# feinanshan/TDNet

Measured on AMD Instinct MI355X. Metric: frames/sec (td4-psp18, 1024x2048, full-resolution logits), higher is better.
Workload: dtype f32; 1 GPU; td4-psp18, 1024x2048 Cityscapes-shaped synthetic stream, 3-frame feature cache, 1 clip per GPU; parallelism=clip-parallel x1, RCCL weight broadcast only, target_fps_per_gpu=30

## Files before the change

include/tdnet.h:

```cpp
#ifndef TDNET_H
#define TDNET_H

#include <stddef.h>
#include <stdint.h>

#ifdef __cplusplus
extern "C" {
#endif

typedef struct tdnet tdnet_t;

typedef struct tdnet_cfg {
    int32_t model;
    int32_t backbone;
    int32_t nclass;
    int32_t height;
    int32_t width;
    int32_t device;
} tdnet_cfg;

#define TDNET_WINOGRAD_DEFAULT 3
#define TDNET_ATTENTION_DEFAULT 2
#define TDNET_FUSION_LN_STATS 2
#define TDNET_FUSION_LN_IN_HEAD 4
#define TDNET_FUSION_A_DIRECT 32
#define TDNET_FUSION_DMA_LOADERS 8192
#define TDNET_FUSION_DMA_NARROW 32768
#define TDNET_FUSION_STEM_ROWS 65536
#define TDNET_FUSION_CONV_GROUPS 131072
#define TDNET_FUSION_CLS_IN_HEAD 262144
#define TDNET_FUSION_SPLIT_NARROW 524288
#define TDNET_FUSION_LATE_CHAIN 1048576
#define TDNET_FUSION_PPM_FOLD 2097152
#define TDNET_OVERLAP_CHAINS 1
#define TDNET_OVERLAP_LOWREG_TRANSFORMS 2
#define TDNET_OVERLAP_CHAINS_ANY_SIZE 4
#define TDNET_OVERLAP_GEMM_DMA 8
#define TDNET_OVERLAP_VW_SHIFT 4
#define TDNET_OVERLAP_VW_MASK 0x30
#define TDNET_FUSION_DEFAULT (TDNET_FUSION_LN_STATS | TDNET_FUSION_LN_IN_HEAD | TDNET_FUSION_A_DIRECT | TDNET_FUSION_DMA_LOADERS | TDNET_FUSION_DMA_NARROW | \
                              TDNET_FUSION_STEM_ROWS | TDNET_FUSION_CONV_GROUPS | TDNET_FUSION_CLS_IN_HEAD | TDNET_FUSION_SPLIT_NARROW | TDNET_FUSION_LATE_CHAIN | TDNET_FUSION_PPM_FOLD)
#define TDNET_FUSION_MASK TDNET_FUSION_DEFAULT
#define TDNET_OVERLAP_DEFAULT (TDNET_OVERLAP_CHAINS | TDNET_OVERLAP_GEMM_DMA | (2 << TDNET_OVERLAP_VW_SHIFT))
#define TDNET_OVERLAP_MASK (TDNET_OVERLAP_CHAINS | TDNET_OVERLAP_LOWREG_TRANSFORMS | TDNET_OVERLAP_CHAINS_ANY_SIZE | TDNET_OVERLAP_GEMM_DMA | TDNET_OVERLAP_VW_MASK)
typedef struct tdnet_opts {
    int32_t winograd;
    int32_t precision;
    int32_t pipeline;
    int32_t gemm_persistent;
    int32_t reserved0;
    int32_t attention;
    int32_t fusion;
    int32_t overlap;
    int32_t reserved[8];
} tdnet_opts;
void tdnet_opts_default(tdnet_opts* o);

typedef struct tdnet_arch {
    int32_t dilated;
    int32_t multi_grid;
    int32_t reserved[6];
} tdnet_arch;
void tdnet_arch_default(tdnet_arch* a);

int  tdnet_create(const tdnet_cfg* cfg, tdnet_t** out);
int  tdnet_create_opts(const tdnet_cfg* cfg, const tdnet_opts* opts , tdnet_t** out);
int  tdnet_create_arch(const tdnet_cfg* cfg, const tdnet_arch* arch , const tdnet_opts* opts ,
                       tdnet_t** out);
int  tdnet_get_opts(const tdnet_t* h, tdnet_opts* out);
int  tdnet_get_arch(const tdnet_t* h, tdnet_arch* out);
int  tdnet_feature_dims(const tdnet_t* h, int* height, int* width);
void tdnet_destroy(tdnet_t* h);

int  tdnet_set_weight(tdnet_t* h, const char* name, const float* host, size_t count);
int  tdnet_finalize_weights(tdnet_t* h);
int  tdnet_create_shared(const tdnet_t* weights_of, const tdnet_opts* opts , tdnet_t** out);
int  tdnet_warmup(tdnet_t* h, void* stream);
int  tdnet_memory_bytes(const tdnet_t* h, size_t* weights_bytes, size_t* handle_bytes);

int  tdnet_forward(tdnet_t* h, const float* img_nchw_dev, int pos_id, float* logits_nchw_dev, void* stream);
int  tdnet_argmax(tdnet_t* h, const float* logits_nchw_dev, int32_t* labels_dev, void* stream);
int  tdnet_forward_labels(tdnet_t* h, const float* img_nchw_dev, int pos_id, int32_t* labels_dev, void* stream);
int  tdnet_set_input_u8(tdnet_t* h, int src_height, int src_width, const double* mean , const double* std );
int  tdnet_forward_u8(tdnet_t* h, const uint8_t* img_hwc_dev, int pos_id, float* logits_nchw_dev, void* stream);
int  tdnet_forward_u8_labels(tdnet_t* h, const uint8_t* img_hwc_dev, int pos_id, uint8_t* labels_dev , void* stream);
int  tdnet_argmax_u8(tdnet_t* h, const float* logits_nchw_dev, uint8_t* labels_dev, void* stream);
#define TDNET_YUV_BT601_LIMITED 0
#define TDNET_YUV_BT709_LIMITED 1
#define TDNET_YUV_BT601_FULL 2
#define TDNET_YUV_BT709_FULL 3
int  tdnet_set_input_nv12(tdnet_t* h, int src_height, int src_width, int pitch, size_t uv_offset, int standard,
                          const double* mean , const double* std );
#define TDNET_PIX_RGB24  0
#define TDNET_PIX_BGR24  1
// ... 65 lines not shown
```

tdnet_amd/_capi.py:

```python
import ctypes
import os

_HERE = os.path.dirname(os.path.abspath(__file__))
DEFAULT_LIB = os.path.join(_HERE, "lib", "libtdnet_hip.so")
TEST_LIB = os.path.join(_HERE, "lib", "libtdnet_hip_test.so")

c_float_p = ctypes.POINTER(ctypes.c_float)
c_void_p = ctypes.c_void_p


class TdnetCfg(ctypes.Structure):
    _fields_ = [("model", ctypes.c_int32), ("backbone", ctypes.c_int32), ("nclass", ctypes.c_int32),
                ("height", ctypes.c_int32), ("width", ctypes.c_int32), ("device", ctypes.c_int32)]


class TdnetOpts(ctypes.Structure):
    _fields_ = [("winograd", ctypes.c_int32), ("precision", ctypes.c_int32), ("pipeline", ctypes.c_int32),
                ("gemm_persistent", ctypes.c_int32), ("reserved0", ctypes.c_int32), ("attention", ctypes.c_int32),
                ("fusion", ctypes.c_int32), ("overlap", ctypes.c_int32), ("reserved", ctypes.c_int32 * 8)]

    def as_dict(self):
        return {k: getattr(self, k) for k, _ in self._fields_ if not k.startswith("reserved")}


# ... 46 lines not shown
    "tdnet_forward_u8": (ctypes.c_int, [c_void_p, c_void_p, ctypes.c_int, c_void_p, c_void_p]),
    "tdnet_forward_u8_labels": (ctypes.c_int, [c_void_p, c_void_p, ctypes.c_int, c_void_p, c_void_p]),
    "tdnet_argmax_u8": (ctypes.c_int, [c_void_p, c_void_p, c_void_p, c_void_p]),
    "tdnet_encode_u8": (ctypes.c_int, [c_void_p, c_void_p, ctypes.c_int, c_void_p]),
    "tdnet_propagate_labels_u8": (ctypes.c_int, [c_void_p, c_void_p, c_void_p]),
    "tdnet_set_output_rgb": (ctypes.c_int, [c_void_p, ctypes.c_int, ctypes.c_int, c_void_p, ctypes.c_int]),
    "tdnet_forward_rgb": (ctypes.c_int, [c_void_p, c_void_p, ctypes.c_int, c_void_p, c_void_p]),
    "tdnet_forward_u8_rgb": (ctypes.c_int, [c_void_p, c_void_p, ctypes.c_int, c_void_p, c_void_p]),
    "tdnet_labels_rgb": (ctypes.c_int, [c_void_p, c_void_p, c_void_p, c_void_p]),
    "tdnet_propagate_rgb": (ctypes.c_int, [c_void_p, c_void_p, c_void_p]),
    "tdnet_set_output_overlay": (ctypes.c_int, [c_void_p, c_void_p, ctypes.c_int]),
    "tdnet_forward_u8_overlay": (ctypes.c_int, [c_void_p, c_void_p, ctypes.c_int, c_void_p, c_void_p]),
    "tdnet_labels_overlay": (ctypes.c_int, [c_void_p, c_void_p, c_void_p, c_void_p, c_void_p]),
    "tdnet_propagate_overlay": (ctypes.c_int, [c_void_p, c_void_p, c_void_p, c_void_p]),
    "tdnet_set_output_view": (ctypes.c_int, [c_void_p, c_view_p]),
    "tdnet_set_score": (ctypes.c_int, [c_void_p, c_void_p]),
    "tdnet_forward_score": (ctypes.c_int, [c_void_p, c_void_p, ctypes.c_int, c_void_p, c_void_p, c_void_p]),
    "tdnet_forward_u8_score": (ctypes.c_int, [c_void_p, c_void_p, ctypes.c_int, c_void_p, c_void_p, c_void_p]),
    "tdnet_propagate_score": (ctypes.c_int, [c_void_p, c_void_p, c_void_p, c_void_p]),
    "tdnet_labels_score": (ctypes.c_int, [c_void_p, c_void_p, c_void_p, c_void_p]),
    "tdnet_score_reset": (ctypes.c_int, [c_void_p, c_void_p]),
    "tdnet_score_export": (ctypes.c_int, [c_void_p, c_void_p, c_void_p]),
    "tdnet_score_read": (ctypes.c_long, [c_void_p, c_void_p, ctypes.c_size_t, c_void_p]),
    "tdnet_set_confidence": (ctypes.c_int, [c_void_p, ctypes.c_int, ctypes.c_int]),
    "tdnet_forward_labels_conf": (ctypes.c_int, [c_void_p, c_void_p, ctypes.c_int, c_void_p, c_void_p, c_void_p]),
    "tdnet_forward_u8_labels_conf": (ctypes.c_int, [c_void_p, c_void_p, ctypes.c_int, c_void_p, c_void_p, c_void_p]),
    "tdnet_propagate_labels_conf": (ctypes.c_int, [c_void_p, c_void_p, c_void_p, c_void_p]),
    "tdnet_logits_conf": (ctypes.c_int, [c_void_p, c_void_p, c_void_p, c_void_p, c_void_p]),
    "tdnet_reset": (ctypes.c_int, [c_void_p]),
    "tdnet_fifo_len": (ctypes.c_int, [c_void_p]),
    "tdnet_encode": (ctypes.c_int, [c_void_p, c_void_p, ctypes.c_int, c_void_p]),
    "tdnet_propagate": (ctypes.c_int, [c_void_p, c_void_p, c_void_p]),
    "tdnet_propagate_labels": (ctypes.c_int, [c_void_p, c_void_p, c_void_p]),
    "tdnet_cache_dims": (ctypes.c_int, [c_void_p, ctypes.POINTER(ctypes.c_int), ctypes.POINTER(ctypes.c_int), ctypes.POINTER(ctypes.c_int)]),
    "tdnet_cache_export": (ctypes.c_int, [c_void_p, c_void_p, c_void_p, c_void_p, c_void_p]),
    "tdnet_cache_push": (ctypes.c_int, [c_void_p, c_void_p, c_void_p, c_void_p, c_void_p]),
    "tdnet_get_stage": (ctypes.c_long, [c_void_p, ctypes.c_char_p, c_void_p, ctypes.c_size_t]),
    "tdnet_flops_per_frame": (ctypes.c_double, [c_void_p]),
    "tdnet_set_profiling": (ctypes.c_int, [c_void_p, ctypes.c_int]),
    "tdnet_last_ms": (ctypes.c_double, [c_void_p, ctypes.c_int]),
    "tdnet_last_flops": (ctypes.c_double, [c_void_p, ctypes.c_int]),
    "tdnet_last_launches": (ctypes.c_double, [c_void_p, ctypes.c_int]),
    "tdnet_last_error": (ctypes.c_char_p, []),
    "tdnet_version": (ctypes.c_char_p, []),
}


TEST_SYMBOLS = {
    "tdnet_bench_mfma_peak": (ctypes.c_double, [ctypes.c_int, ctypes.c_int, c_void_p]),
    "tdnet_bench_conv": (ctypes.c_double, [ctypes.c_int] * 9 + [c_opts_p, c_void_p]),
    "tdnet_op_conv2d": (ctypes.c_int, [c_void_p, ctypes.c_int, ctypes.c_int, ctypes.c_int, c_void_p, c_void_p, ctypes.c_int,
                                       ctypes.c_int, ctypes.c_int, ctypes.c_int, c_void_p, ctypes.c_int, c_opts_p, ctypes.c_int,
                                       c_void_p, c_void_p]),
    "tdnet_op_conv2d_f16io": (ctypes.c_int, [c_void_p, ctypes.c_int, ctypes.c_int, ctypes.c_int, c_void_p, c_void_p, ctypes.c_int,
                                             ctypes.c_int, ctypes.c_int, ctypes.c_int, c_void_p, ctypes.c_int, ctypes.c_int,
                                             c_void_p, c_void_p]),
    "tdnet_op_conv2d_f16mix": (ctypes.c_int, [c_void_p, ctypes.c_int, ctypes.c_int, ctypes.c_int, c_void_p, c_void_p, ctypes.c_int,
                                              ctypes.c_int, ctypes.c_int, ctypes.c_int, c_void_p, ctypes.c_int, ctypes.c_int, ctypes.c_int,
                                              ctypes.c_int, c_void_p, c_void_p]),
    "tdnet_op_conv_group_f16": (ctypes.c_int, [ctypes.c_int] + [c_void_p] * 12 + [ctypes.c_int] * 4 + [ctypes.POINTER(ctypes.c_int), c_void_p]),
    "tdnet_op_cache_subsample": (ctypes.c_int, [c_void_p, c_void_p] + [ctypes.c_int] * 4 + [c_void_p, c_void_p, c_void_p]),
    "tdnet_op_conv1x1_rows": (ctypes.c_int, [c_void_p, ctypes.c_int, ctypes.c_int, ctypes.c_int, c_void_p, c_void_p, ctypes.c_int, ctypes.c_int,
                                             c_opts_p, ctypes.c_int, ctypes.c_int, c_void_p, c_void_p]),
    "tdnet_op_maxpool": (ctypes.c_int, [c_void_p, ctypes.c_int, ctypes.c_int, ctypes.c_int, ctypes.c_int, c_void_p, c_void_p]),
    "tdnet_op_stem_f16": (ctypes.c_int, [c_void_p, ctypes.c_int, ctypes.c_int, c_void_p, c_void_p, ctypes.c_int, c_void_p, c_void_p]),
    "tdnet_op_stem": (ctypes.c_int, [c_void_p, ctypes.c_int, ctypes.c_int, c_void_p, c_void_p, c_opts_p, c_void_p, c_void_p]),
    "tdnet_op_attention": (ctypes.c_int, [c_void_p, c_void_p, c_void_p, c_void_p, c_void_p, ctypes.c_int, ctypes.c_int,
                                          ctypes.c_int, ctypes.c_int, c_void_p, c_void_p, c_void_p, c_void_p, c_void_p]),
    "tdnet_op_layernorm_hw": (ctypes.c_int, [c_void_p, ctypes.c_int, ctypes.c_int, c_void_p, c_void_p, c_void_p, c_void_p]),
    "tdnet_op_layernorm_hw_f16": (ctypes.c_int, [c_void_p, ctypes.c_int, ctypes.c_int, c_void_p, c_void_p, c_void_p, c_void_p]),
    "tdnet_op_ppm": (ctypes.c_int, [c_void_p, ctypes.c_int, ctypes.c_int, c_void_p, c_void_p, ctypes.c_int, ctypes.c_int,
                                    c_void_p, c_void_p]),
    "tdnet_op_upsample": (ctypes.c_int, [c_void_p, ctypes.c_int, ctypes.c_int, ctypes.c_int, ctypes.c_int, ctypes.c_int,
                                         c_void_p, c_void_p]),
    "tdnet_op_stem_image": (ctypes.c_long, [c_void_p, c_void_p, ctypes.c_int, ctypes.c_int, ctypes.c_int, ctypes.c_int, ctypes.POINTER(ctypes.c_double),
                                            ctypes.POINTER(ctypes.c_double), ctypes.c_int, c_void_p, ctypes.c_size_t, c_void_p]),
    "tdnet_op_stem_image_nv12": (ctypes.c_long, [c_void_p, ctypes.c_int, ctypes.c_int, ctypes.c_int, ctypes.c_size_t, ctypes.c_int, ctypes.c_int, ctypes.c_int,
                                                 ctypes.POINTER(ctypes.c_double), ctypes.POINTER(ctypes.c_double), ctypes.c_int, c_void_p, ctypes.c_size_t, c_void_p]),
    "tdnet_op_stem_image_view": (ctypes.c_long, [c_void_p, c_view_p, ctypes.c_int, ctypes.c_int, ctypes.POINTER(ctypes.c_double), ctypes.POINTER(ctypes.c_double),
                                                 ctypes.c_int, c_void_p, ctypes.c_size_t, c_void_p]),
    "tdnet_op_overlay_view": (ctypes.c_int, [c_void_p] + [ctypes.c_int] * 5 + [c_void_p, c_void_p, c_view_p, c_void_p, ctypes.c_int, c_void_p, c_void_p]),
    "tdnet_op_picture_view": (ctypes.c_int, [c_void_p] + [ctypes.c_int] * 5 + [c_void_p, c_void_p, ctypes.c_int, c_void_p, c_view_p, ctypes.c_int, ctypes.c_int,
                                             c_void_p, c_view_p, c_void_p]),
    "tdnet_op_upsample_argmax": (ctypes.c_int, [c_void_p, ctypes.c_int, ctypes.c_int, ctypes.c_int, ctypes.c_int, ctypes.c_int, c_void_p, c_void_p, c_void_p]),
    "tdnet_op_upsample_argmax_rgb": (ctypes.c_int, [c_void_p] + [ctypes.c_int] * 7 + [c_void_p, ctypes.c_int, c_void_p, c_void_p, c_void_p]),
    "tdnet_op_overlay": (ctypes.c_int, [c_void_p] + [ctypes.c_int] * 5 + [c_void_p, c_void_p] + [ctypes.c_int] * 4 + [ctypes.c_size_t, ctypes.c_int, c_void_p, ctypes.c_int,
                                        c_void_p, c_void_p]),
    "tdnet_op_upsample_argmax_score": (ctypes.c_int, [c_void_p] + [ctypes.c_int] * 5 + [c_void_p] * 6),
    "tdnet_op_upsample_argmax_conf": (ctypes.c_int, [c_void_p] + [ctypes.c_int] * 5 + [c_void_p, c_void_p, ctypes.c_int, ctypes.c_int, c_void_p, c_void_p]),
    "tdnet_op_nearest_index": (ctypes.c_int, [ctypes.c_int, ctypes.c_int, c_void_p]),
    "tdnet_op_enc_first": (ctypes.c_int, [c_void_p] + [ctypes.c_int] * 4 + [c_void_p] * 4 + [ctypes.c_int] + [c_void_p] * 4 + [ctypes.c_int] + [c_void_p] * 5),
    "tdnet_op_conv1x1_src2_null": (ctypes.c_int, [c_void_p, ctypes.c_int, ctypes.c_int, ctypes.c_int, c_void_p, c_void_p, ctypes.c_int, ctypes.c_int,
                                                  c_void_p, ctypes.c_int, c_opts_p, ctypes.c_int, c_void_p, c_void_p]),
    "tdnet_op_classifier": (ctypes.c_int, [c_void_p, ctypes.c_int, ctypes.c_int, c_void_p, c_void_p, ctypes.c_int, c_void_p, c_void_p]),
    "tdnet_op_head_cls": (ctypes.c_int, [c_void_p, ctypes.c_int, ctypes.c_int, ctypes.c_int, c_void_p, c_void_p, ctypes.c_int, ctypes.c_int,
                                         c_void_p, c_void_p, ctypes.c_int, c_opts_p, ctypes.c_int, c_void_p, c_void_p]),
}


class Lib:

    def __init__(self, path=DEFAULT_LIB, test_symbols=False):
        if not os.path.exists(path):
            raise TdnetError("HIP library not found: %s -- build it with `python -c 'import __graft_entry__ as g; g.build()'` "
                             "(hipcc --offload-arch=gfx950); there is no CPU fallback" % path)
        self.path = path
# ... 48 lines not shown
```

tdnet_amd/csrc/td_handle.h:

```cpp
#pragma once
#include "../../include/tdnet.h"
#include "td_device.h"
#include "td_conv.h"
#include "td_conv_h.h"
#include "td_conv_hd.h"
#include "td_conv_ad.h"
#include "td_wino.h"
#include "td_gemm.h"
#include "td_gemm_dma.h"
#include "td_gemm_b3.h"
#include "td_conv_ad_b3.h"
#include "td_attn.h"
#include "td_attn_h.h"
#include "td_attn_b3.h"
#include "td_misc.h"
#include "td_ingest.h"
#include "td_out.h"
#include "td_score.h"
#include "td_conf.h"

#include <cmath>
#include <cstdarg>
#include <cstdio>
#include <algorithm>
#include <atomic>
#include <cstring>
#include <cstdlib>
#include <map>
#include <string>
#include <vector>

static thread_local char g_err[1024] = "";
static int td_fail(const char* fmt, ...) {
    va_list ap;
    va_start(ap, fmt);
    vsnprintf(g_err, sizeof(g_err), fmt, ap);
    va_end(ap);
    return -1;
}
#define TD_HIP(expr)                                                                            \
    do {                                                                                        \
        hipError_t e_ = (expr);                                                                 \
        if (e_ != hipSuccess) return td_fail("%s failed: %s (%s:%d)", #expr, hipGetErrorString(e_), __FILE__, __LINE__); \
    } while (0)

#define TD_TRY(expr) do { if ((expr) != 0) return -1; } while (0)

struct DevGuard {
    int prev = -1;
    bool switched = false, ok = true;
    explicit DevGuard(int dev) {
        if (hipGetDevice(&prev) != hipSuccess) { ok = false; return; }
        if (prev != dev) { ok = hipSetDevice(dev) == hipSuccess; switched = ok; }
    }
    ~DevGuard() { if (switched) (void)hipSetDevice(prev); }
};
#define TD_ON_DEVICE(n, ...)                                                                      \
    DevGuard dev_guard_((n)->cfg.device);                                                         \
    if (!dev_guard_.ok) { td_fail("cannot select HIP device %d", (n)->cfg.device); return __VA_ARGS__; }

// ... 3 lines not shown
    const int nb18[4] = {2, 2, 2, 2}, nb34[4] = {3, 4, 6, 3};
    const int nb101[4] = {3, 4, 23, 3};
    const int* nb = backbone == 18 ? nb18 : backbone == 101 ? nb101 : nb34;
    const bool bott = backbone == 50 || backbone == 101;
    const int exp = bott ? 4 : 1;
    const int planes[4] = {64, 128, 256, 512};
    const int strides[4] = {1, 2, dilated ? 1 : 2, dilated ? 1 : 2}, dils[4] = {1, 1, dilated ? 2 : 1, dilated ? 4 : 1};
    std::vector<BlockSpec> out;
    int inpl = bott ? 128 : 64;
    for (int li = 0; li < 4; ++li) {
        for (int b = 0; b < nb[li]; ++b) {
            const bool first = b == 0, mg = li == 3 && dilated && multi_grid;
            int d1;
            if (mg) d1 = b == 0 ? 4 : b == 1 ? 8 : 16;
            else if (first) d1 = (dils[li] == 1 || dils[li] == 2) ? 1 : 2;
            else d1 = dils[li];
            BlockSpec s;
            char nm[32];
            snprintf(nm, sizeof(nm), "layer%d.%d", li + 1, b);
            s.name = nm;
            s.cin = first ? inpl : planes[li] * exp;
            s.cout = planes[li] * exp;
            s.bott = bott;
            s.planes = planes[li];
            s.stride = first ? strides[li] : 1;
            s.dil1 = d1;
            s.dil2 = dils[li];
            s.ds = first && (strides[li] != 1 || inpl != planes[li] * exp);
            out.push_back(s);
        }
        inpl = planes[li] * exp;
    }
    return out;
}
static int key_size(int n) { return (n - 1) / 4 + 1; }
static int out_size(int n, int KS, int stride, int dil, int pad) { return (n + 2 * pad - dil * (KS - 1) - 1) / stride + 1; }
static int feature_size(int n, const std::vector<BlockSpec>& blocks) {
    n = (n - 1) / 2 + 1;
    n = (n - 1) / 2 + 1;
    for (const BlockSpec& s : blocks) n = out_size(n, 3, s.stride, s.dil1, s.dil1);
    return n;
}

enum ConvRoute {
    CR_IGEMM,
    CR_ADIRECT,
    CR_ADIRECT_ROWS,
    CR_ADIRECT_B3,
    CR_ADIRECT_ROWS_B3,
    CR_GEMM1X1,
    CR_STEM_H,
    CR_CONV_H,
    CR_CONV_DMA,
    CR_WINO
};
enum GemmKernel {
    GK_CONV,
    GK_PERSISTENT,
    GK_DMA,
    GK_B3
};
struct ConvLayer {
    int Cin = 0, Cout = 0, KS = 1, stride = 1, dil = 1, pad = 0, act = 0;
    bool stem = false;
    ConvRoute route = CR_IGEMM;
    GemmKernel gemm = GK_CONV;
    bool in16 = false, out16 = false;
    int rh = 0;
    bool rowimg_off = false;
    int pers = 1;
    int chunks = 1;
    int vw = 0;
    int wino = 0;
    float* d_zero = nullptr;
    ConvTile tile = CT_128x128;
    int CoutPad = 0, nsteps = 0;
    float* d_wp = nullptr;
    float* d_bias = nullptr;
    bool h16() const { return route == CR_STEM_H || route == CR_CONV_H || route == CR_CONV_DMA; }
    bool stem_rows() const { return route == CR_ADIRECT_ROWS || route == CR_ADIRECT_ROWS_B3; }
    double flops_per_pixel() const { return 2.0 * Cout * (stem ? 3.0 * KS * KS : (double)Cin * KS * KS); }
};

static_assert(TDNET_FUSION_DEFAULT == 4169766 && TDNET_FUSION_MASK == 4169766 && TDNET_OVERLAP_DEFAULT == 41 && TDNET_OVERLAP_MASK == 0x3f,
              "the named option bits of include/tdnet.h must add up to the documented values");
static tdnet_opts opts_or_default(const tdnet_opts* o) {
    tdnet_opts d;
    tdnet_opts_default(&d);
    if (!o) return d;
    d = *o;
    d.winograd = d.winograd <= 0 ? 0 : (d.winograd == 2 || d.winograd >= 4) ? 4 : 3;
    d.precision = d.precision < 0 ? 0 : d.precision > 3 ? 1 : d.precision;
    d.pipeline = d.pipeline ? 1 : 0;
    d.gemm_persistent = d.gemm_persistent < 0 ? 0 : d.gemm_persistent;
    d.attention = d.attention < 0 ? 0 : d.attention > 2 ? 2 : d.attention;
    d.fusion &= TDNET_FUSION_MASK;
    d.overlap = d.overlap < 0 ? 0 : d.overlap & TDNET_OVERLAP_MASK;
    if ((d.overlap & TDNET_OVERLAP_VW_MASK) == TDNET_OVERLAP_VW_MASK) d.overlap &= ~TDNET_OVERLAP_VW_MASK;
    d.reserved0 = 0;
    for (int& r : d.reserved) r = 0;
    return d;
}

struct BlockLayers { ConvLayer c1, c2, c3, ds; bool has_ds = false, bott = false; };
struct AtnLayer { ConvLayer fc; float* d_bias = nullptr; };
struct PathLayers {
    ConvLayer stem, stem2, stem3;
    std::vector<BlockLayers> blocks;
    float* d_ppm_w = nullptr; float* d_ppm_b = nullptr;
    ConvLayer enc_v, enc_q0, enc_q1, enc_k0, enc_k1;
    std::vector<AtnLayer> atn;
    float* d_ln_g = nullptr; float* d_ln_b = nullptr;
    ConvLayer head3;
    float* d_cls_w = nullptr; float* d_cls_b = nullptr;
    int pid = 0;
};
struct CacheSlot { float* q = nullptr; float* k = nullptr; float* v = nullptr; };
struct Nv12Layout { int pitch; size_t uv_offset; int standard; };
struct SrcView {
    int format = 0;
    int fh = 0, fw = 0, pitch = 0, oy = 0, ox = 0;
    size_t uv_offset = 0;
    int standard = 0;
};
static SrcView src_view_rgb(int Hs, int Ws) { SrcView v; v.fh = Hs; v.fw = Ws; return v; }
static SrcView src_view_nv12(int Hs, int Ws, const Nv12Layout& nv) {
    SrcView v; v.format = TDNET_PIX_NV12; v.fh = Hs; v.fw = Ws; v.pitch = nv.pitch; v.uv_offset = nv.uv_offset; v.standard = nv.standard; return v;
}
static int src_view_bpp(int format) { return format == TDNET_PIX_NV12 ? 1 : format >= TDNET_PIX_RGBA32 ? 4 : 3; }
struct U8Input {
    bool set = false;
    bool nv12 = false;
    int format = 0, bpp = 3;
    bool swap = false;
    int fh = 0, fw = 0, oy = 0, ox = 0;
    int pitch = 0, standard = 0, span_c = 0;
    size_t uv_offset = 0, extent = 0;
// ... 471 lines not shown
```

tdnet_amd/csrc/td_launch.h:

```cpp
#pragma once
#include "td_weights.h"

#ifdef TDNET_TIMING_PROBES
static int probe_skip() {
    static const int m = [] {
        const char* e = getenv("TDNET_PROBE_SKIP");
        const int v = e ? atoi(e) : 0;
        if (v) fprintf(stderr, "tdnet: TDNET_PROBE_SKIP=%d -- pieces of the frame are NOT computed, every result of this process is garbage (timing probe build)\n", v);
        return v;
    }();
    return m;
}
#else
static constexpr int probe_skip() { return 0; }
#endif
static void prof_begin(tdnet* n, int family, int dominant, double flops, hipStream_t s) {
    if (!n || !n->prof) return;
    if (n->nrec == n->recs.size()) {
        ProfRec r;
        hipEventCreate(&r.e0); hipEventCreate(&r.e1);
        n->recs.push_back(r);
    }
    ProfRec& r = n->recs[n->nrec];
    r.family = family; r.dominant = dominant; r.flops = flops;
// ... 74 lines not shown
            if (L.Cout == 128) TD_LAUNCH((k_wino4_out_cls<2>), dim3(grid), dim3(256), wino_out_cls_lds(128, cls->NC), s, wa, *cls);
            else TD_LAUNCH((k_wino4_out_cls<1>), dim3(grid), dim3(256), wino_out_cls_lds(64, cls->NC), s, wa, *cls);
        } else
        if (L.vw == 1) launch_wino4_c<1>(out_side, wa, s);
        else if (L.vw == 2 && C % 2 == 0) launch_wino4_c<2>(out_side, wa, s);
        else if (L.vw == 4 && C % 4 == 0) launch_wino4_c<4>(out_side, wa, s);
        else if (L.vw) launch_wino4_c<1>(out_side, wa, s);
        else if (out_side && wino_act_general(wa.act)) TD_LAUNCH((k_wino4_out<true>), dim3(td_grid_for(T * (L.Cout / 4), 256, 256 * 16)), dim3(256), 0, s, wa);
        else if (out_side) TD_LAUNCH((k_wino4_out<false>), dim3(td_grid_for(T * (L.Cout / 4), 256, 256 * 16)), dim3(256), 0, s, wa);
        else TD_LAUNCH(k_wino4_in, dim3(td_grid_for(T * (L.Cin / 4), 256, 256 * 16)), dim3(256), 0, s, wa);
        prof_end(n, s);
    };
    transform(false);
    prof_begin(n, 0, 2, 2.0 * nb * Tc * (double)L.Cin * L.Cout, s);
    if (!(n && (probe_skip() & 8))) launch_gemm(L, gemm_args(L, V, (int)Tc, nb, L.d_zero, nullptr, Mb, 0), chunked ? 320 : 0, s);
    prof_end(n, s);
    transform(true);
    if (own) { TD_HIP(hipStreamSynchronize(s)); hipFree(V); hipFree(Mb); }
    return 0;
}

static void launch_conv_dma_forms(const ConvLayer& L, const ConvArgs& a, hipStream_t s) {
    int rh = L.rh;
    bool done = false;
    const bool is192 = rh == CD_192_P || rh == CD_192_N;
    if (rh == CD_128_N || rh == CD_192_N) {
        done = !L.rowimg_off && conv_launch_dma3n(a, rh, L.KS, L.out16, s);
        if (!done) rh = is192 ? CD_192_P : CD_128_P;
    }
    if (!done && (rh == CD_128_P || rh == CD_192_P)) {
        done = !L.rowimg_off && conv_launch_dma3p(a, rh, L.KS, L.out16, s);
        if (!done) rh = is192 ? CD_192 : CD_128_8W;
    }
    if (!done && (L.rowimg_off || !conv_launch_dma3(a, rh, L.KS, L.out16, s))) conv_launch_dma(a, rh, L.KS, L.out16, s);
}

static int run_conv(tdnet* n, const ConvLayer& L, const float* in, int H, int W, const float* resid, float* out, hipStream_t s,
                    int* Ho_out = nullptr, int* Wo_out = nullptr, const LnFuse* lnf = nullptr, const ClsArgs* cls = nullptr) {
    if (lnf && !L.wino) return td_fail("internal: LayerNorm fusion needs a Winograd input transform");
    if (cls && (!L.wino || L.chunks > 1 || resid || wino_act_general(L.act))) return td_fail("internal: the classifier rides in a whole Winograd conv's output transform");
    const int Ho = out_size(H, L.KS, L.stride, L.dil, L.pad), Wo = out_size(W, L.KS, L.stride, L.dil, L.pad);
    if (L.wino) {
        if (Ho_out) *Ho_out = H;
        if (Wo_out) *Wo_out = W;
        if (L.chunks > 1 && (!n || !n->ws_ready)) {
            for (int c = 0; c < L.chunks; ++c) {
                WinoChunk ck; ck.ny = L.chunks; ck.cy = c;
                TD_TRY(run_wino(n, L, in, H, W, resid, out, s, lnf, ck, nullptr, nullptr));
            }
            return 0;
        }
        return run_wino(n, L, in, H, W, resid, out, s, lnf, WinoChunk(), nullptr, nullptr, cls);
    }
    const ConvArgs a = conv_args(L, in, H, W, resid, out);
    prof_begin(n, 0, (((L.tile == CT_128x128 || L.tile == CT_128x128_DEEP || L.rh) && L.KS == 3 && !L.stem) ? 1 : 0) | ((L.h16() && L.in16 && L.KS == 3 && !L.stem) ? 4 : 0), L.flops_per_pixel() * a.M, s);
    switch (L.route) {
    case CR_STEM_H: conv_launch_stem_h(a, L.out16, s); break;
    case CR_CONV_DMA: launch_conv_dma_forms(L, a, s); break;
    case CR_CONV_H: conv_launch_h(a, L.tile, L.KS, L.in16, L.out16, s); break;
    case CR_ADIRECT_B3: conv_launch_adirect_b3(a, L.KS, 0, s); break;
    case CR_GEMM1X1: launch_gemm(L, gemm_args(L, in, a.M, 1, L.d_bias, resid, out, L.act), 0, s); break;
    case CR_ADIRECT_ROWS:
    case CR_ADIRECT_ROWS_B3: {
        ConvArgs r = a;
        r.H = stem_rows_hp(H); r.W = stem_rows_wp(W); r.Cin = 3; r.pad = 0;
        if (L.route == CR_ADIRECT_ROWS_B3) conv_launch_adirect_b3(r, L.KS, 2, s);
        else conv_launch_adirect(r, L.KS, 2, s);
        break;
    }
    case CR_ADIRECT: conv_launch_adirect(a, L.KS, L.stem ? 1 : 0, s); break;
    case CR_IGEMM: conv_launch(a, L.tile, L.KS, L.stem, s); break;
    case CR_WINO: break;
    }
    prof_end(n, s);
    if (Ho_out) *Ho_out = Ho;
    if (Wo_out) *Wo_out = Wo;
    return 0;
}

static int run_conv_src2(tdnet* n, const ConvLayer& L, const float* in, int ld, int k_split, int nsteps, const float* in2, int ld2, const float* wp2,
                         int H, int W, const float* resid, float* out, hipStream_t s) {
    if (L.KS != 1 || L.stem || L.wino) return td_fail("internal: two operand sources need a 1x1 conv");
    const ConvArgs a0 = conv_args(L, in, H, W, resid, out);
    prof_begin(n, 0, 0, 2.0 * L.Cout * 32.0 * nsteps * a0.M, s);
    int rc = 0;
    if (L.route == CR_GEMM1X1 && L.gemm == GK_PERSISTENT) {
        GemmArgs ga = gemm_args(L, in, a0.M, 1, L.d_bias, resid, out, L.act);
        ga.K = 32 * nsteps; ga.k_split = k_split; ga.lda = ld; ga.a2 = in2; ga.lda2 = ld2; ga.wp2 = wp2;
        if (!gemm_src2_supports(ga)) rc = td_fail("internal: the persistent GEMM cannot take this second operand source");
        else launch_gemm(L, ga, 0, s);
    } else if (L.route == CR_ADIRECT) {
        ConvArgs a = a0;
        a.Cin = 32 * nsteps; a.nsteps = nsteps; a.k_split = k_split; a.ld = ld; a.in2 = in2; a.ld2 = ld2; a.wp2 = wp2;
        if (resid || !conv_adirect_src2_supports(a, L.KS, 0)) rc = td_fail("internal: the direct 1x1 conv cannot take this second operand source");
        else conv_launch_adirect(a, 1, 0, s);
    } else rc = td_fail("internal: this conv's kernel has no second operand source");
    prof_end(n, s);
    return rc;
}

struct ConvCall { const ConvLayer* L; const float* in; int H, W; float* out; };
static bool conv_group_same_form(const tdnet_opts& o, const ConvCall* c, int ng) {
    bool same = (o.fusion & TDNET_FUSION_CONV_GROUPS) && ng >= 2 && ng <= 3;
    for (int g = 0; same && g < ng; ++g) {
        const ConvLayer& L = *c[g].L;
        const ConvLayer& L0 = *c[0].L;
        same = L.route == CR_CONV_H && L.in16 == L.out16 && L.in16 == L0.in16 && (g == 0 ? (L.KS == 1 || L.KS == 3) : L.KS == 1) &&
               conv_tile_dims(L.tile).BM == conv_tile_dims(L0.tile).BM && conv_tile_dims(L.tile).BN == conv_tile_dims(L0.tile).BN;
    }
    return same;
}
static int run_conv_group(tdnet* n, const tdnet_opts& o, const ConvCall* c, int ng, hipStream_t s, int* Ho_out = nullptr, int* Wo_out = nullptr,
                          int* grouped = nullptr) {
    const bool same = conv_group_same_form(o, c, ng);
    if (grouped) *grouped = same ? 1 : 0;
    if (!same) {
        for (int g = 0; g < ng; ++g) TD_TRY(run_conv(n, *c[g].L, c[g].in, c[g].H, c[g].W, nullptr, c[g].out, s, g == 0 ? Ho_out : nullptr, g == 0 ? Wo_out : nullptr));
        return 0;
    }
    ConvArgs a[3];
    double flops = 0.0;
    for (int g = 0; g < ng; ++g) {
        const ConvLayer& L = *c[g].L;
        a[g] = conv_args(L, c[g].in, c[g].H, c[g].W, nullptr, c[g].out);
// ... 329 lines not shown
```

tdnet_amd/csrc/td_weights.h:

```cpp
#pragma once
#include "td_handle.h"

constexpr int RH_FRAME = -1;
constexpr int RH_BY_SIZE = -2;

static int plan_dma_form(const ConvLayer& c, long M, const tdnet_opts& o) {
    const bool narrow = (o.fusion & TDNET_FUSION_DMA_NARROW) != 0, same3 = c.KS == 3 && c.stride == 1 && c.pad == c.dil;
    if (!conv_dma_supports(c.Cin, c.Cout, c.KS, c.tile)) return CD_NONE;
    if (c.Cout == 64 && c.CoutPad == 128 && same3 && narrow) return CD_128_N;
    if (c.Cout < 128) return CD_NONE;
    const int rh = conv_dma_pick_rh(M, c.Cout, c.CoutPad % 256 == 0);
    if (narrow && same3 && M <= 16384 && c.Cout <= 256) return c.Cout <= 128 ? CD_128_N : CD_192_N;
    if (o.fusion & TDNET_FUSION_DMA_LOADERS) return rh == CD_128 ? CD_128_P : rh == CD_192 ? CD_192_P : rh;
    return rh;
}

static int plan_conv(ConvLayer& L, int Cout, int Cin, int KS, int stride, int dil, int act, bool stem, long M, const tdnet_opts& o,
                     int forced_tile = -1, int chunks = 1, bool in16 = false, bool out16 = false, int rh = RH_FRAME, bool rowimg_off = false) {
    L = ConvLayer();
    L.Cin = stem ? 4 : Cin; L.Cout = Cout; L.KS = KS; L.stride = stride; L.dil = dil; L.act = act; L.stem = stem;
    L.pad = stem ? KS / 2 : dil * (KS / 2);
    L.pers = o.gemm_persistent;
    L.rowimg_off = rowimg_off;
    if (!stem && Cin % 32 != 0) return td_fail("conv: Cin=%d is not a multiple of 32", Cin);
    const bool deep = o.pipeline != 0, forced = forced_tile >= 0;
    const bool pers_gemm = o.gemm_persistent && gemm_supports(Cin);
    const bool split = o.precision >= 2;
    const bool split_narrow = split && (o.fusion & TDNET_FUSION_A_DIRECT) && (o.fusion & TDNET_FUSION_SPLIT_NARROW);
    if (o.winograd && o.precision != 1 && !stem && KS == 3 && stride == 1 && Cin % 32 == 0 && Cout % 4 == 0 && (o.winograd == 4 || (Cin >= 128 && Cout >= 128))) {
        L.route = CR_WINO;
        L.wino = 4;
        L.chunks = (chunks > 1 && dil % chunks == 0 && pers_gemm) ? chunks : 1;
        L.vw = (L.chunks > 1 || (o.overlap & TDNET_OVERLAP_LOWREG_TRANSFORMS)) ? (1 << ((o.overlap & TDNET_OVERLAP_VW_MASK) >> TDNET_OVERLAP_VW_SHIFT)) : 0;
        const int nb = (L.wino + 2) * (L.wino + 2);
        const long rows = wino_tiles_estimate(M, dil, L.wino) / L.chunks;
        L.tile = forced ? (ConvTile)forced_tile : pers_gemm ? gemm_pick_tile(rows, nb, Cout, deep)
                                                            : conv_pick_tile((int)std::min<long>(nb * M / (L.wino * L.wino), 1 << 30), Cout, deep);
        L.nsteps = conv_nsteps(Cin, 1, 0);
        const bool b3 = split && pers_gemm && gemm_b3_supports(Cin, Cout) && (forced || o.precision == 3 || gemm_b3_pick(rows, nb, Cout));
        L.gemm = !pers_gemm ? GK_CONV : b3 ? GK_B3 : ((o.overlap & TDNET_OVERLAP_GEMM_DMA) && gemm_dma_supports(Cin, Cout, L.tile)) ? GK_DMA : GK_PERSISTENT;
        L.CoutPad = b3 ? gemm_b3_npad(Cout) : conv_cout_pad(Cout, L.tile);
        return 0;
    }
    const bool h16 = o.precision == 1 && !stem && Cin % 64 == 0;
    const bool stem16 = o.precision == 1 && stem && KS == 7 && stride == 2 && Cout <= 64;
    const bool is1x1 = !h16 && !stem && KS == 1 && stride == 1 && pers_gemm;
    const bool narrow1x1 = is1x1 && !forced && split_narrow && Cout <= 128 && M >= 8192 && gemm_b3_supports(Cin, Cout) && !gemm_b3_pick(M, 1, Cout, Cin) &&
                           conv_adirect_b3_supports(CT_128x64, Cin, KS, stem);
    const bool gemm1x1 = is1x1 && !narrow1x1;
    L.tile = forced ? (ConvTile)forced_tile : gemm1x1 ? gemm_pick_tile(M, 1, Cout, deep) : conv_pick_tile((int)M, Cout, deep);
    if (!forced && split_narrow && !h16 && !stem && !gemm1x1 && Cout <= 128 && conv_adirect_b3_supports(CT_128x64, Cin, KS, stem)) L.tile = CT_128x64;
    if (h16 && !forced && (o.fusion & TDNET_FUSION_DMA_NARROW) && KS == 3 && stride == 1 && Cout == 64) L.tile = CT_128x128_DEEP;
    L.CoutPad = conv_cout_pad(Cout, L.tile);
    L.nsteps = conv_nsteps(Cin, KS, stem ? 1 : 0);
    if (stem16 && conv_stem_h_supports(L.tile)) {
        L.route = CR_STEM_H;
        L.nsteps = conv_nsteps_stem_h();
    } else if (h16) {
        L.route = CR_CONV_H;
        L.nsteps = conv_nsteps_h(Cin, KS);
    } else if (gemm1x1) {
        const bool b3 = split && gemm_b3_supports(Cin, Cout) && (forced || o.precision == 3 || gemm_b3_pick(M, 1, Cout, Cin));
        L.route = CR_GEMM1X1;
        L.gemm = b3 ? GK_B3 : GK_PERSISTENT;
        if (b3) { L.CoutPad = gemm_b3_npad(Cout); L.nsteps = Cin / 16; }
    } else if (split_narrow && conv_adirect_b3_supports(L.tile, Cin, KS, stem)) {
        L.route = CR_ADIRECT_B3;
    } else if ((o.fusion & TDNET_FUSION_A_DIRECT) && conv_adirect_supports(L.tile, 1)) {
        const bool rows = stem && KS == 7 && stride == 2 && (o.fusion & TDNET_FUSION_STEM_ROWS);
        L.route = !rows ? CR_ADIRECT : split_narrow ? CR_ADIRECT_ROWS_B3 : CR_ADIRECT_ROWS;
        if (rows) L.nsteps = conv_nsteps(Cin, KS, 2);
    }
    if (L.h16()) { L.in16 = in16; L.out16 = out16; }
    if (L.route == CR_CONV_H && L.in16) {
        L.rh = rh == RH_FRAME ? plan_dma_form(L, M, o)
             : rh == RH_BY_SIZE ? (Cout >= 128 && conv_dma_supports(Cin, Cout, KS, L.tile) ? conv_dma_pick_rh(M, Cout, L.CoutPad % 256 == 0) : CD_NONE) : rh;
        if (L.rh) L.route = CR_CONV_DMA;
    }
    return 0;
}

static bool plan_enc_fold(const tdnet_opts& o, const ConvLayer& v, const ConvLayer& q0, const ConvLayer& k0, int XS, int FS) {
    const auto gemm = [](const ConvLayer& L) { return L.route == CR_GEMM1X1 && L.gemm == GK_PERSISTENT; };
    return (o.fusion & TDNET_FUSION_PPM_FOLD) && o.precision == 0 && gemm(v) && gemm(q0) && k0.route == CR_ADIRECT && k0.KS == 1 && !k0.stem &&
           XS >= 64 && XS % 64 == 0 && FS % 16 == 0 && v.Cin == XS + 4 * FS && q0.Cin == v.Cin && k0.Cin == v.Cin &&
           v.CoutPad % 64 == 0 && q0.CoutPad % 64 == 0 && k0.CoutPad % 64 == 0;
}

template <typename T, typename Pack>
static int upload_packed(float** d, size_t count, Pack pack) {
    std::vector<T> packed(count);
    pack(packed.data());
    TD_TRY(dev_alloc((T**)d, count));
    TD_HIP(hipMemcpy(*d, packed.data(), count * sizeof(T), hipMemcpyHostToDevice));
    return 0;
}
static int upload_conv(ConvLayer& L, const std::vector<float>& w, const std::vector<float>& b) {
    typedef unsigned short bf16;
    const int Cout = L.Cout, Cin = L.Cin, KS = L.KS, stem_kind = L.stem_rows() ? 2 : L.stem ? 1 : 0;
    const size_t tile_image = (size_t)L.nsteps * 8 * L.CoutPad * 4;
    if (L.route == CR_WINO) {
        const int nb = (L.wino + 2) * (L.wino + 2);
        std::vector<std::vector<float>> U;
        wino_transform_weights(w.data(), Cout, Cin, L.wino, U);
        const size_t per = L.gemm == GK_B3 ? gemm_b3_packed_bytes(Cin, Cout) / 2 : tile_image;
        if (L.gemm == GK_B3) TD_TRY(upload_packed<bf16>(&L.d_wp, nb * per, [&](bf16* p) { for (int bi = 0; bi < nb; ++bi) gemm_b3_pack(U[bi].data(), Cout, Cin, p + bi * per); }));
        else TD_TRY(upload_packed<float>(&L.d_wp, nb * per, [&](float* p) { for (int bi = 0; bi < nb; ++bi) conv_pack_weights(U[bi].data(), Cout, Cin, 1, 0, L.tile, p + bi * per); }));
    } else if (L.route == CR_STEM_H)
        TD_TRY(upload_packed<_Float16>(&L.d_wp, 2 * tile_image, [&](_Float16* p) { conv_pack_weights_stem_h(w.data(), Cout, L.tile, p); }));
    else if (L.h16())
        TD_TRY(upload_packed<_Float16>(&L.d_wp, 2 * tile_image, [&](_Float16* p) { conv_pack_weights_h(w.data(), Cout, Cin, KS, L.tile, p); }));
    else if (L.route == CR_GEMM1X1 && L.gemm == GK_B3)
        TD_TRY(upload_packed<bf16>(&L.d_wp, gemm_b3_packed_bytes(Cin, Cout) / 2, [&](bf16* p) { gemm_b3_pack(w.data(), Cout, Cin, p); }));
    else if (L.route == CR_ADIRECT_B3 || L.route == CR_ADIRECT_ROWS_B3)
        TD_TRY(upload_packed<bf16>(&L.d_wp, conv_adb3_packed_bytes(Cout, Cin, KS, stem_kind) / 2, [&](bf16* p) { conv_pack_weights_adb3(w.data(), Cout, Cin, KS, p, stem_kind); }));
    else
        TD_TRY(upload_packed<float>(&L.d_wp, tile_image, [&](float* p) { conv_pack_weights(w.data(), Cout, Cin, KS, stem_kind, L.tile, p); }));
    TD_TRY(upload(&L.d_bias, b.empty() ? std::vector<float>(Cout, 0.f) : b));
    if (L.wino) TD_TRY(upload(&L.d_zero, std::vector<float>(Cout, 0.f)));
    return 0;
}
static void free_conv_layer(ConvLayer& L) {
    if (L.d_wp) hipFree(L.d_wp);
    if (L.d_bias) hipFree(L.d_bias);
    if (L.d_zero) hipFree(L.d_zero);
    L.d_wp = L.d_bias = L.d_zero = nullptr;
}
static void add_bn(std::map<std::string, size_t>& e, const std::string& pre, int c) {
    e[pre + ".weight"] = c; e[pre + ".bias"] = c; e[pre + ".running_mean"] = c; e[pre + ".running_var"] = c;
    e[pre + ".num_batches_tracked"] = 1;
}
static std::vector<std::string> atn_module_names(int model) {
    if (model == 4) return {"atn1_2", "atn1_3", "atn1_4", "atn2_1", "atn2_3", "atn2_4", "atn3_1", "atn3_2", "atn3_4", "atn4_1", "atn4_2", "atn4_3"};
    return {"atn1", "atn2"};
}
static std::vector<std::string> atn_order(int model, int p) {
    if (model == 2) return {p == 0 ? "atn1" : "atn2"};
    static const char* t[4][3] = {{"atn1_2", "atn1_3", "atn1_4"}, {"atn2_3", "atn2_4", "atn2_1"},
                                  {"atn3_4", "atn3_1", "atn3_2"}, {"atn4_1", "atn4_2", "atn4_3"}};
    return {t[p][0], t[p][1], t[p][2]};
}
static void build_expected(tdnet* n) {
    auto& e = n->expected;
    char b[160];
    for (int p = 1; p <= n->P; ++p) {
        snprintf(b, sizeof(b), "pretrained%d", p);
        std::string pre = n->cfg.model == 1 ? std::string("pretrained") : std::string(b);
        if (n->deep) {
            e[pre + ".conv1.0.weight"] = 64 * 3 * 9; add_bn(e, pre + ".conv1.1", 64);
            e[pre + ".conv1.3.weight"] = 64 * 64 * 9; add_bn(e, pre + ".conv1.4", 64);
            e[pre + ".conv1.6.weight"] = 128 * 64 * 9; add_bn(e, pre + ".bn1", 128);
        } else {
            e[pre + ".conv1.weight"] = 64 * 3 * 49;
            add_bn(e, pre + ".bn1", 64);
        }
        for (auto& s : n->bspec) {
            std::string bp = pre + "." + s.name;
            if (s.bott) {
                e[bp + ".conv1.weight"] = (size_t)s.planes * s.cin; add_bn(e, bp + ".bn1", s.planes);
                e[bp + ".conv2.weight"] = (size_t)s.planes * s.planes * 9; add_bn(e, bp + ".bn2", s.planes);
                e[bp + ".conv3.weight"] = (size_t)s.cout * s.planes; add_bn(e, bp + ".bn3", s.cout);
// ... 387 lines not shown
```

Baseline: 293.1 frames/s.

## Add fused single-kernel Winograd F(4,3) path for 64-channel 3x3 convolutions

Adds a new conv route that runs the whole Winograd F(4x4,3x3) convolution for 64-in/64-out 3x3 stride-1 layers in one kernel. The kernel does the input transform into LDS, MFMA batched products against prepacked transformed weights, and the output transform with bias, residual and activation. This replaces the multi-kernel Winograd or implicit-GEMM path and is meant to cut the intermediate transform-buffer traffic and launch overhead on the large early-stage maps. It is enabled by default for fp32 when the map is large enough. The risk is the heavy register and LDS use (nine 16-wide accumulators per thread), which may limit occupancy.

```diff
diff --git a/include/tdnet.h b/include/tdnet.h
--- a/include/tdnet.h
+++ b/include/tdnet.h
@@ -32,6 +32,7 @@
 #define TDNET_FUSION_SPLIT_NARROW 524288
 #define TDNET_FUSION_LATE_CHAIN 1048576
 #define TDNET_FUSION_PPM_FOLD 2097152
+#define TDNET_FUSION_WINO_F64 4194304
 #define TDNET_OVERLAP_CHAINS 1
 #define TDNET_OVERLAP_LOWREG_TRANSFORMS 2
 #define TDNET_OVERLAP_CHAINS_ANY_SIZE 4
@@ -39,7 +40,8 @@
 #define TDNET_OVERLAP_VW_SHIFT 4
 #define TDNET_OVERLAP_VW_MASK 0x30
 #define TDNET_FUSION_DEFAULT (TDNET_FUSION_LN_STATS | TDNET_FUSION_LN_IN_HEAD | TDNET_FUSION_A_DIRECT | TDNET_FUSION_DMA_LOADERS | TDNET_FUSION_DMA_NARROW | \
-                              TDNET_FUSION_STEM_ROWS | TDNET_FUSION_CONV_GROUPS | TDNET_FUSION_CLS_IN_HEAD | TDNET_FUSION_SPLIT_NARROW | TDNET_FUSION_LATE_CHAIN | TDNET_FUSION_PPM_FOLD)
+                              TDNET_FUSION_STEM_ROWS | TDNET_FUSION_CONV_GROUPS | TDNET_FUSION_CLS_IN_HEAD | TDNET_FUSION_SPLIT_NARROW | TDNET_FUSION_LATE_CHAIN | TDNET_FUSION_PPM_FOLD | \
+                              TDNET_FUSION_WINO_F64)
 #define TDNET_FUSION_MASK TDNET_FUSION_DEFAULT
 #define TDNET_OVERLAP_DEFAULT (TDNET_OVERLAP_CHAINS | TDNET_OVERLAP_GEMM_DMA | (2 << TDNET_OVERLAP_VW_SHIFT))
 #define TDNET_OVERLAP_MASK (TDNET_OVERLAP_CHAINS | TDNET_OVERLAP_LOWREG_TRANSFORMS | TDNET_OVERLAP_CHAINS_ANY_SIZE | TDNET_OVERLAP_GEMM_DMA | TDNET_OVERLAP_VW_MASK)
diff --git a/tdnet_amd/_capi.py b/tdnet_amd/_capi.py
--- a/tdnet_amd/_capi.py
+++ b/tdnet_amd/_capi.py
@@ -122,6 +122,8 @@
     "tdnet_op_conv2d": (ctypes.c_int, [c_void_p, ctypes.c_int, ctypes.c_int, ctypes.c_int, c_void_p, c_void_p, ctypes.c_int,
                                        ctypes.c_int, ctypes.c_int, ctypes.c_int, c_void_p, ctypes.c_int, c_opts_p, ctypes.c_int,
                                        c_void_p, c_void_p]),
+    "tdnet_op_conv_wino_f64": (ctypes.c_int, [c_void_p, ctypes.c_int, ctypes.c_int, ctypes.c_int, c_void_p, c_void_p, ctypes.c_int,
+                                              ctypes.c_int, ctypes.c_int, ctypes.c_int, c_void_p, ctypes.c_int, c_void_p, c_void_p]),
     "tdnet_op_conv2d_f16io": (ctypes.c_int, [c_void_p, ctypes.c_int, ctypes.c_int, ctypes.c_int, c_void_p, c_void_p, ctypes.c_int,
                                              ctypes.c_int, ctypes.c_int, ctypes.c_int, c_void_p, ctypes.c_int, ctypes.c_int,
                                              c_void_p, c_void_p]),
diff --git a/tdnet_amd/csrc/td_handle.h b/tdnet_amd/csrc/td_handle.h
--- a/tdnet_amd/csrc/td_handle.h
+++ b/tdnet_amd/csrc/td_handle.h
@@ -6,6 +6,7 @@
 #include "td_conv_hd.h"
 #include "td_conv_ad.h"
 #include "td_wino.h"
+#include "td_wino_f64.h"
 #include "td_gemm.h"
 #include "td_gemm_dma.h"
 #include "td_gemm_b3.h"
@@ -115,7 +116,8 @@
     CR_STEM_H,
     CR_CONV_H,
     CR_CONV_DMA,
-    CR_WINO
+    CR_WINO,
+    CR_WINO_F64
 };
 enum GemmKernel {
     GK_CONV,
@@ -145,7 +147,7 @@
     double flops_per_pixel() const { return 2.0 * Cout * (stem ? 3.0 * KS * KS : (double)Cin * KS * KS); }
 };
 
-static_assert(TDNET_FUSION_DEFAULT == 4169766 && TDNET_FUSION_MASK == 4169766 && TDNET_OVERLAP_DEFAULT == 41 && TDNET_OVERLAP_MASK == 0x3f,
+static_assert(TDNET_FUSION_DEFAULT == 8364070 && TDNET_FUSION_MASK == 8364070 && TDNET_OVERLAP_DEFAULT == 41 && TDNET_OVERLAP_MASK == 0x3f,
               "the named option bits of include/tdnet.h must add up to the documented values");
 static tdnet_opts opts_or_default(const tdnet_opts* o) {
     tdnet_opts d;
diff --git a/tdnet_amd/csrc/td_launch.h b/tdnet_amd/csrc/td_launch.h
--- a/tdnet_amd/csrc/td_launch.h
+++ b/tdnet_amd/csrc/td_launch.h
@@ -150,8 +150,10 @@
         }
         return run_wino(n, L, in, H, W, resid, out, s, lnf, WinoChunk(), nullptr, nullptr, cls);
     }
+    if (L.route == CR_WINO_F64 && !wino_f64_size_ok(H, W)) return td_fail("internal: this map is too large for the fused Winograd kernel");
     const ConvArgs a = conv_args(L, in, H, W, resid, out);
-    prof_begin(n, 0, (((L.tile == CT_128x128 || L.tile == CT_128x128_DEEP || L.rh) && L.KS == 3 && !L.stem) ? 1 : 0) | ((L.h16() && L.in16 && L.KS == 3 && !L.stem) ? 4 : 0), L.flops_per_pixel() * a.M, s);
+    const double flops = L.route == CR_WINO_F64 ? 2.0 * 36 * (double)wino_tiles(H, W, 1, 4) * L.Cin * L.Cout : L.flops_per_pixel() * a.M;
+    prof_begin(n, 0, (((L.tile == CT_128x128 || L.tile == CT_128x128_DEEP || L.rh) && L.KS == 3 && !L.stem) ? 1 : 0) | ((L.h16() && L.in16 && L.KS == 3 && !L.stem) ? 4 : 0), flops, s);
     switch (L.route) {
     case CR_STEM_H: conv_launch_stem_h(a, L.out16, s); break;
     case CR_CONV_DMA: launch_conv_dma_forms(L, a, s); break;
@@ -168,6 +170,7 @@
     }
     case CR_ADIRECT: conv_launch_adirect(a, L.KS, L.stem ? 1 : 0, s); break;
     case CR_IGEMM: conv_launch(a, L.tile, L.KS, L.stem, s); break;
+    case CR_WINO_F64: wino_f64_launch(in, L.d_wp, L.d_bias, resid, out, H, W, L.act, s); break;
     case CR_WINO: break;
     }
     prof_end(n, s);
diff --git a/tdnet_amd/csrc/td_weights.h b/tdnet_amd/csrc/td_weights.h
--- a/tdnet_amd/csrc/td_weights.h
+++ b/tdnet_amd/csrc/td_weights.h
@@ -13,6 +13,11 @@
     if (narrow && same3 && M <= 16384 && c.Cout <= 256) return c.Cout <= 128 ? CD_128_N : CD_192_N;
     if (o.fusion & TDNET_FUSION_DMA_LOADERS) return rh == CD_128 ? CD_128_P : rh == CD_192 ? CD_192_P : rh;
     return rh;
+}
+
+static bool plan_wino_f64(const tdnet_opts& o, int Cout, int Cin, int KS, int stride, int dil, int act, bool stem, bool forced_tile, int chunks) {
+    return (o.fusion & TDNET_FUSION_WINO_F64) && o.winograd >= 3 && o.precision == 0 && !forced_tile && chunks == 1 &&
+           wino_f64_supports(Cout, Cin, KS, stride, dil, act, stem);
 }
 
 static int plan_conv(ConvLayer& L, int Cout, int Cin, int KS, int stride, int dil, int act, bool stem, long M, const tdnet_opts& o,
@@ -27,6 +32,11 @@
     const bool pers_gemm = o.gemm_persistent && gemm_supports(Cin);
     const bool split = o.precision >= 2;
     const bool split_narrow = split && (o.fusion & TDNET_FUSION_A_DIRECT) && (o.fusion & TDNET_FUSION_SPLIT_NARROW);
+    if (plan_wino_f64(o, Cout, Cin, KS, stride, dil, act, stem, forced, chunks) && M >= TD_WINO_F64_MIN_PIXELS && M <= TD_WINO_F64_MAX_PIXELS) {
+        L.route = CR_WINO_F64;
+        L.nsteps = 0; L.CoutPad = Cout;
+        return 0;
+    }
     if (o.winograd && o.precision != 1 && !stem && KS == 3 && stride == 1 && Cin % 32 == 0 && Cout % 4 == 0 && (o.winograd == 4 || (Cin >= 128 && Cout >= 128))) {
         L.route = CR_WINO;
         L.wino = 4;
@@ -106,7 +116,9 @@
         const size_t per = L.gemm == GK_B3 ? gemm_b3_packed_bytes(Cin, Cout) / 2 : tile_image;
         if (L.gemm == GK_B3) TD_TRY(upload_packed<bf16>(&L.d_wp, nb * per, [&](bf16* p) { for (int bi = 0; bi < nb; ++bi) gemm_b3_pack(U[bi].data(), Cout, Cin, p + bi * per); }));
         else TD_TRY(upload_packed<float>(&L.d_wp, nb * per, [&](float* p) { for (int bi = 0; bi < nb; ++bi) conv_pack_weights(U[bi].data(), Cout, Cin, 1, 0, L.tile, p + bi * per); }));
-    } else if (L.route == CR_STEM_H)
+    } else if (L.route == CR_WINO_F64)
+        TD_TRY(upload_packed<float>(&L.d_wp, wino_f64_packed_floats(), [&](float* p) { wino_f64_pack(w.data(), p); }));
+    else if (L.route == CR_STEM_H)
         TD_TRY(upload_packed<_Float16>(&L.d_wp, 2 * tile_image, [&](_Float16* p) { conv_pack_weights_stem_h(w.data(), Cout, L.tile, p); }));
     else if (L.h16())
         TD_TRY(upload_packed<_Float16>(&L.d_wp, 2 * tile_image, [&](_Float16* p) { conv_pack_weights_h(w.data(), Cout, Cin, KS, L.tile, p); }));
diff --git a/tdnet_amd/csrc/td_wino_f64.h b/tdnet_amd/csrc/td_wino_f64.h
--- /dev/null
+++ b/tdnet_amd/csrc/td_wino_f64.h
@@ -0,0 +1,174 @@
+#pragma once
+#include "td_wino.h"
+
+constexpr int TD_WF64_C = 64;
+constexpr int TD_WF64_BX = 8, TD_WF64_BY = 4;
+constexpr int TD_WF64_LDS = 36 * 8 * 2 * 32 * 4;
+constexpr long TD_WINO_F64_MIN_PIXELS = 32768;
+
+struct WinoF64Args {
+    const float* in;
+    const float* up;
+    const float* bias;
+    const float* resid;
+    float* out;
+    int H, W, BXN, act;
+};
+
+static inline bool wino_f64_supports(int Cout, int Cin, int KS, int stride, int dil, int act, bool stem) {
+    return !stem && KS == 3 && stride == 1 && dil == 1 && Cin == TD_WF64_C && Cout == TD_WF64_C && (act == 0 || act == 1);
+}
+constexpr long TD_WINO_F64_MAX_PIXELS = (1l << 31) / (TD_WF64_C * 4) - 1;
+static inline bool wino_f64_size_ok(int H, int W) { return H >= 1 && W >= 1 && (long)H * W <= TD_WINO_F64_MAX_PIXELS; }
+constexpr int TD_WF64_PACKED_FLOATS = 2 * 36 * 8 * 64 * 4;
+static inline size_t wino_f64_packed_floats() { return (size_t)TD_WF64_PACKED_FLOATS; }
+static inline void wino_f64_pack(const float* w, float* p) {
+    std::vector<std::vector<float>> U;
+    wino_transform_weights(w, TD_WF64_C, TD_WF64_C, 4, U);
+    for (int hb = 0; hb < 2; ++hb)
+        for (int pos = 0; pos < 36; ++pos)
+            for (int kq = 0; kq < 8; ++kq)
+                for (int lane = 0; lane < 64; ++lane)
+                    for (int j = 0; j < 4; ++j)
+                        p[((((size_t)hb * 36 + pos) * 8 + kq) * 64 + lane) * 4 + j] =
+                            U[pos][(size_t)(32 * hb + (lane & 31)) * TD_WF64_C + 8 * kq + 4 * (lane >> 5) + j];
+}
+
+TD_DEV int td_wf64_vidx(int pos, int slot, int tile) { return pos * 512 + slot * 32 + (tile ^ (4 * ((slot >> 2) & 3))); }
+TD_DEV int td_wf64_midx(int pos, int j, int t) { return pos * 512 + j * 16 + (t ^ (2 * (j >> 2))); }
+
+TD_KERNEL void TD_LAUNCH_BOUNDS(256, 2) k_wino4_f64(WinoF64Args p) {
+    TD_DYN_LDS(smem);
+    float* lds = reinterpret_cast<float*>(smem);
+    const int tid = threadIdx.x, lane = tid & 63, wave = TD_UNIFORM(tid >> 6);
+    const int bx = (int)blockIdx.x % p.BXN, by = (int)blockIdx.x / p.BXN, hb = (int)blockIdx.y;
+    const unsigned map_bytes = (unsigned)p.H * (unsigned)p.W * (unsigned)TD_WF64_C * 4u;
+    const TdBuf inb = td_make_buf(p.in, map_bytes);
+    const TdBuf ub = td_make_buf(p.up, (unsigned)TD_WF64_PACKED_FLOATS * 4u);
+    const TdBuf rb = td_make_buf(p.resid, p.resid ? map_bytes : 0u);
+    const TdBuf ob = td_make_buf(p.out, map_bytes);
+    f32x16 acc[9];
+#pragma unroll
+    for (int q = 0; q < 9; ++q)
+#pragma unroll
+        for (int r = 0; r < 16; ++r) acc[q][r] = 0.f;
+    const unsigned ulane = (unsigned)lane * 16u;
+    const unsigned ubase = (unsigned)((hb * 36 + wave * 9) * 8) * 1024u;
+    const float* va[4];
+#pragma unroll
+    for (int g = 0; g < 4; ++g) va[g] = lds + td_wf64_vidx(wave * 9, 4 * g + (lane >> 5), lane & 31);
+
+#pragma unroll 1
+    for (int kc = 0; kc < 4; ++kc) {
+        int t = tid;
+        TD_PIN(t);
+        const int tl = t >> 3, cp = t & 7;
+        const int tx = bx * TD_WF64_BX + (tl & 7), ty = by * TD_WF64_BY + (tl >> 3);
+        unsigned offy[6], offx[6];
+#pragma unroll
+        for (int r = 0; r < 6; ++r) {
+            const int y = 4 * ty - 1 + r, x = 4 * tx - 1 + r;
+            offy[r] = (unsigned)y < (unsigned)p.H ? (unsigned)y * (unsigned)p.W * (unsigned)(TD_WF64_C * 4) : TD_BUF_OOB;
+            offx[r] = (unsigned)x < (unsigned)p.W ? (unsigned)x * (unsigned)(TD_WF64_C * 4) + (unsigned)(16 * kc + 2 * cp) * 4u : TD_BUF_OOB;
+        }
+        f32x2 dd[6][6];
+#pragma unroll
+        for (int c = 0; c < 6; ++c)
+#pragma unroll
+            for (int r = 0; r < 6; ++r) dd[c][r] = td_buf_ld2(inb, __builtin_elementwise_add_sat(offy[r], offx[c]), 0u);
+        f32x2 tm[6][6];
+#pragma unroll
+        for (int c = 0; c < 6; ++c) {
+            f32x2 col[6];
+            td_wino4_bt_t(dd[c], col);
+#pragma unroll
+            for (int r = 0; r < 6; ++r) tm[r][c] = col[r];
+        }
+        if (kc) __syncthreads();
+        float* vd = lds + td_wf64_vidx(0, (4 * (cp >> 2) + ((2 * cp) & 3)) * 2 + ((cp >> 1) & 1), tl);
+#pragma unroll
+        for (int r = 0; r < 6; ++r) {
+            f32x2 v[6];
+            td_wino4_bt_t(tm[r], v);
+#pragma unroll
+            for (int c = 0; c < 6; ++c) {
+                vd[(r * 6 + c) * 512] = v[c][0];
+                vd[(r * 6 + c) * 512 + 64] = v[c][1];
+            }
+        }
+        f32x4 b0[9], b1[9];
+#pragma unroll
+        for (int q = 0; q < 9; ++q) b0[q] = td_buf_ld4(ub, ulane, ubase + (unsigned)((q * 8 + 2 * kc) * 1024));
+        __syncthreads();
+#pragma unroll
+        for (int q = 0; q < 9; ++q) b1[q] = td_buf_ld4(ub, ulane, ubase + (unsigned)((q * 8 + 2 * kc + 1) * 1024));
+#pragma unroll
+        for (int j = 0; j < 4; ++j)
+#pragma unroll
+            for (int q = 0; q < 9; ++q) acc[q] = td_mfma32(va[j >> 1][q * 512 + (j & 1) * 64], b0[q][j], acc[q]);
+#pragma unroll
+        for (int j = 0; j < 4; ++j)
+#pragma unroll
+            for (int q = 0; q < 9; ++q) acc[q] = td_mfma32(va[2 + (j >> 1)][q * 512 + (j & 1) * 64], b1[q][j], acc[q]);
+    }
+
+    const int tl = tid >> 4, cpp = tid & 15;
+    const TdBuf bb = td_make_buf(p.bias, (unsigned)(TD_WF64_C * 4));
+    const f32x2 b = td_buf_ld2(bb, (unsigned)(32 * hb + 2 * cpp) * 4u, 0u);
+#pragma unroll
+    for (int rd = 0; rd < 2; ++rd) {
+        const int tx = bx * TD_WF64_BX + (tl & 7), ty = by * TD_WF64_BY + 2 * rd + (tl >> 3);
+        unsigned offy[4], offx[4];
+#pragma unroll
+        for (int r = 0; r < 4; ++r) {
+            const int y = 4 * ty + r, x = 4 * tx + r;
+            offy[r] = y < p.H ? (unsigned)y * (unsigned)p.W * (unsigned)(TD_WF64_C * 4) : TD_BUF_OOB;
+            offx[r] = x < p.W ? (unsigned)x * (unsigned)(TD_WF64_C * 4) + (unsigned)(32 * hb + 2 * cpp) * 4u : TD_BUF_OOB;
+        }
+        f32x2 o[16];
+#pragma unroll
+        for (int r = 0; r < 4; ++r)
+#pragma unroll
+            for (int c = 0; c < 4; ++c) o[r * 4 + c] = td_buf_ld2(rb, __builtin_elementwise_add_sat(offy[r], offx[c]), 0u);
+        __syncthreads();
+        {
+            const int j = lane & 31, i4 = 4 * (lane >> 5);
+#pragma unroll
+            for (int q = 0; q < 9; ++q)
+#pragma unroll
+                for (int r = 0; r < 8; ++r) lds[td_wf64_midx(wave * 9 + q, j, (r & 3) + 8 * (r >> 2) + i4)] = acc[q][8 * rd + r];
+        }
+        __syncthreads();
+        f32x2 sm[4][6];
+#pragma unroll
+        for (int c = 0; c < 6; ++c) {
+            f32x2 mc[6], col[4];
+#pragma unroll
+            for (int r = 0; r < 6; ++r) mc[r] = f32x2{lds[td_wf64_midx(r * 6 + c, 2 * cpp, tl)], lds[td_wf64_midx(r * 6 + c, 2 * cpp + 1, tl)]};
+            td_wino4_at_t(mc, col);
+#pragma unroll
+            for (int r = 0; r < 4; ++r) sm[r][c] = col[r];
+        }
+#pragma unroll
+        for (int r = 0; r < 4; ++r) {
+            f32x2 o4[4];
+            td_wino4_at_t(sm[r], o4);
+#pragma unroll
+            for (int c = 0; c < 4; ++c) o[r * 4 + c] = (o4[c] + b) + o[r * 4 + c];
+        }
+        td_wino_activate<false>(o, p.act);
+#pragma unroll
+        for (int r = 0; r < 4; ++r)
+#pragma unroll
+            for (int c = 0; c < 4; ++c) td_buf_st2(ob, __builtin_elementwise_add_sat(offy[r], offx[c]), 0u, o[r * 4 + c]);
+    }
+}
+
+static inline bool wino_f64_launch(const float* in, const float* up, const float* bias, const float* resid, float* out, int H, int W, int act, hipStream_t s) {
+    if (!wino_f64_size_ok(H, W)) return false;
+    const int TX = wino_tiles_1d(W, 1, 4), TY = wino_tiles_1d(H, 1, 4);
+    const int bxn = (TX + TD_WF64_BX - 1) / TD_WF64_BX, byn = (TY + TD_WF64_BY - 1) / TD_WF64_BY;
+    const WinoF64Args a = {in, up, bias, resid, out, H, W, bxn, act};
+    TD_LAUNCH(k_wino4_f64, dim3((unsigned)(bxn * byn), 2), dim3(256), TD_WF64_LDS, s, a);
+    return true;
+}
```

After: 303.7 frames/s (median of 6 runs). +3.6%, better.
